# carlobaldassi/RRRMC.jl

Measured on AMD Instinct MI355X. Metric: spin-flip attempts/sec (whole node), GraphRRG N=4096 K=3 +-J standardMC beta=1.0, higher is better.
Workload: dtype u32

## Files before the change

rrrmc.jl_amd/csrc/host_sweep.hpp:

```cpp
int32_t prepare_chunk_list(rrrmc_ctx* ctx, int64_t iters, int64_t step, int C, bool* reuse_out)
{
    const bool reuse = ctx->chunks_iters == iters && ctx->chunks_step == step && ctx->chunks_C == C;
    if (!reuse) {
        std::vector<ChunkDesc> chunks;
        plan_chunk_list(iters, step, C, kWave, ctx->batch_slots_max, ctx->batch_chunks_max, ctx->batch_first_chunks, chunks, ctx->chunk_batches);
        const size_t nch_all = chunks.size();
        ctx->chunks_iters = -1;
        if (ctx->upload_pending) { HIP_TRY(ctx, hipEventSynchronize(ctx->ev_upload)); ctx->upload_pending = false; }
        if (nch_all > ctx->chunks_cap) {
            HIP_TRY(ctx, hipStreamSynchronize(ctx->stream));
            HIP_TRY(ctx, hipStreamSynchronize(ctx->plan_stream));
            free_dev(ctx->d_chunks);
            free_dev(ctx->d_chunks_alt);
            ctx->chunks_cap = 0;
            HIP_TRY(ctx, hipMalloc(&ctx->d_chunks, sizeof(ChunkDesc) * nch_all));
            if (ctx->model == RRRMC_MODEL_SPARSE_PM1) HIP_TRY(ctx, hipMalloc(&ctx->d_chunks_alt, sizeof(ChunkDesc) * nch_all));
            ctx->chunks_cap = nch_all;
        }
        if (nch_all > ctx->h_chunks_cap) {
            if (ctx->h_chunks) { (void)hipHostFree(ctx->h_chunks); ctx->h_chunks = nullptr; }
            ctx->h_chunks_cap = 0;
            HIP_TRY(ctx, hipHostMalloc(&ctx->h_chunks, sizeof(ChunkDesc) * nch_all));
            ctx->h_chunks_cap = nch_all;
        }
// ... 86 lines not shown
        if (nchunks) HIP_TRY(ctx, hipMemcpyAsync(ctx->d_chunks, ctx->h_chunks, sizeof(ChunkDesc) * nchunks, hipMemcpyHostToDevice, st));
        if (nchunks) HIP_TRY(ctx, hipMemcpyAsync(ctx->d_chunks_alt, ctx->h_chunks, sizeof(ChunkDesc) * nchunks, hipMemcpyHostToDevice, st));
        ctx->chunks_iters = iters; ctx->chunks_step = step; ctx->chunks_C = C;
        ctx->upload_pending = true;
    }
    HIP_TRY(ctx, hipEventRecord(ctx->ev_upload, st));
    if (!reuse) HIP_TRY(ctx, hipStreamWaitEvent(ctx->plan_stream, ctx->ev_upload, 0));
    for (int i = 0; i < 2; ++i)
        if (!ctx->ev_set_free[i]) HIP_TRY(ctx, hipEventCreateWithFlags(&ctx->ev_set_free[i], hipEventDisableTiming));
    const int par = ctx->plan_parity;
    auto set_of = [par](int b) -> int { return (b + par) & 1; };
    ChunkDesc* const d_chunks = (ctx->call_parity ^= 1) ? ctx->d_chunks_alt : ctx->d_chunks;

    P.spins = ctx->d_spins;
    P.table = ctx->d_table;
    P.Es = ctx->d_Es;
    P.E_cur = ctx->d_E;
    P.acc_cur = ctx->d_acc;
    P.k0 = (uint32_t)ctx->seed;
    P.k1 = (uint32_t)(ctx->seed >> 32);
    P.group0 = ctx->replica0 / 32;
    P.gbase = ctx->it_done;
    P.N = (int)N; P.C = C; P.TS = ctx->TS; P.Rpad = (int)ctx->Rpad;
    sweep_fn fn = ctx->lds_mode ? sweep_for_K((int)K, ctx->sweep_mode) : nullptr;
    BigSweepParams PB{};
    BigMaskParams PM{};
    if (ctx->big_masks) {
        std::memcpy(PM.taum, P.taum, sizeof(PM.taum));
        PM.always_mask = P.always_mask; PM.k0 = P.k0; PM.k1 = P.k1; PM.group0 = P.group0; PM.gbase = P.gbase;
        PM.cap = (uint32_t)ctx->batch_slots_max;
        PM.lgr = ctx->big_cm ? ctx->big_lgr : -1;
    }
    if (ctx->big_mode) {
        PB.spins = ctx->d_spins; PB.Es = ctx->d_Es; PB.E_cur = ctx->d_E; PB.acc_cur = ctx->d_acc;
        std::memcpy(PB.taum, P.taum, sizeof(PB.taum));
        PB.always_mask = P.always_mask; PB.k0 = P.k0; PB.k1 = P.k1; PB.group0 = P.group0; PB.gbase = P.gbase;
        PB.N = (int)N; PB.Rpad = (int)ctx->Rpad;
    }
#ifdef RRRMC_STAMPS
    if (!g_stamps) HIP_TRY(ctx, hipMalloc(&g_stamps, sizeof(unsigned long long) * 16 * (65536 + 4096)));
    P.stamps = g_stamps;
#endif
    const int nb = (int)batches.size();
    auto launch_plan = [&](int b) -> int32_t {
        const rrrmc_ctx::BatchDesc& bt = batches[b];
        const int set = set_of(b);
        if (ctx->set_used[set]) HIP_TRY(ctx, hipStreamWaitEvent(ctx->plan_stream, ctx->ev_set_free[set], 0));
        if (ctx->big_mode) {
            hipLaunchKernelGGL(plan_big_for_K((int)K), dim3((unsigned)bt.n), dim3(kPlanThreads), ctx->plan_lds_bytes, ctx->plan_stream,
                               d_chunks + bt.first, ctx->d_slots[set], ctx->d_nbrs[set], ctx->d_vecs[set], ctx->d_A, ctx->d_J, (int)N, P.k0, P.k1, P.gbase,
                               ctx->big_masks ? ctx->big_lgr : -1);
            if (ctx->big_masks) {
                PM.chunks = d_chunks + bt.first; PM.slots = ctx->d_slots[set]; PM.masks = ctx->d_masks[set];
                hipLaunchKernelGGL(big_mask_for_K((int)K), dim3((unsigned)(bt.n * (kBigChunk / kBigMaskThreads)), (unsigned)ctx->G), dim3(kBigMaskThreads), 0,
                                   ctx->plan_stream, PM);
            }
        }
        else
            hipLaunchKernelGGL(plan_for_K((int)K), dim3((unsigned)bt.n), dim3(kPlanThreads), ctx->plan_lds_bytes, ctx->plan_stream,
                               d_chunks + bt.first, ctx->d_slots[set], ctx->d_vecs[set], ctx->d_A, (int)N, C, P.k0, P.k1, P.gbase,
                               sweep_rows_for_K((int)K) * kWave);
        HIP_TRY(ctx, hipGetLastError());
        HIP_TRY(ctx, hipEventRecord(ctx->ev_plan[b], ctx->plan_stream));
// ... 48 lines not shown
```

rrrmc.jl_amd/csrc/rrrmc_hip.hip:

```cpp
#include "../../include/rrrmc_hip.h"

#include <hip/hip_runtime.h>

#include <algorithm>
#include <cmath>
#include <cstdarg>
#include <cstdio>
#include <cstdlib>
#include <cstring>
#include <string>
#include <thread>
#include <map>
#include <mutex>
#include <utility>
#include <vector>

#include "sk_kernels.hpp"
#include "sk_block_kernel.hpp"
#include "sk_hblock_kernel.hpp"
#include "rrr_kernels.hpp"
#include "quant_wave_kernel.hpp"
#include "sparse_wave_kernel.hpp"
#include "sparse_kernels.hpp"
#include "bign_kernels.hpp"
// ... 157 lines not shown
    uint32_t* rp_spins = nullptr;
    uint8_t* rp_cls = nullptr;
    uint16_t* rp_sv = nullptr;
    uint16_t* rp_spos = nullptr;
    double* wt_t = nullptr;
    uint16_t* wt_id = nullptr;
    uint16_t* wt_pos = nullptr;
    double* wt_time = nullptr;
    uint32_t wtm_calls = 0;
    bool last_call_wtm = false;
    uint32_t* eo_cmin = nullptr;
    double* eo_ftau = nullptr;
    bool last_call_eo = false;
    double* rs_buf = nullptr;
    uint32_t* rs_spins = nullptr;
    int32_t* rs_status = nullptr;

    double* pf_J = nullptr;
    unsigned long long* pf_spins = nullptr;
    double* pf_undo = nullptr;
    int32_t* pf_sites = nullptr;
    uint32_t* pf_plan = nullptr;
    int32_t* pf_status = nullptr;
    int64_t pfW = 0;
    bool pf_multi_edge = false;
    bool pf_lf_live = false;
    int8_t* db_dJ = nullptr;
    double* db_rJ = nullptr;
    uint8_t* db_cls = nullptr;
    uint16_t* db_sv = nullptr;
    uint16_t* db_spos = nullptr;
    double* db_lf = nullptr;
    double* db_undo = nullptr;
    int db_L = 0, db_ea_form = 0;
    long long db_lev_mul = 1;
    double db_lev_div = 1.0;
    bool db_cache_valid = false;
    bool q_lds_attr = false;
    bool q_cache_valid = false;
    LevTable lv{};
    long long lv_mul = 1;
    double lv_div = 1.0;
    int64_t eo_W = 0;
    int db_dElist[kDLmax] = {0};
    uint32_t* cs_spins = nullptr;
    double* cs_buf = nullptr;
// ... 344 lines not shown
    } while (0)

namespace {
int32_t post_sync_checks(rrrmc_ctx* ctx)
{
    if (ctx->debug_checks && ctx->dbg_flag) {
        int32_t fl[2] = {0, 0};
        HIP_TRY(ctx, hipMemcpy(fl, ctx->dbg_flag, sizeof fl, hipMemcpyDeviceToHost));
        HIP_TRY(ctx, hipMemset(ctx->dbg_flag, 0, sizeof fl));
        if (fl[0])
            return fail(ctx, RRRMC_ERR_STATE, "debug check failed for %d value(s), e.g. replica %d: the tracked energy / cached fields differ from "
                                              "energy(X, C) recomputed from the configuration (src/graphs/RRG.jl:229-231, SK.jl:268-273)", fl[0], fl[1]);
    }
    if (ctx->model == RRRMC_MODEL_SPARSE_F64 && ctx->pf_status && !ctx->last_call_rrr) {
        int32_t st = 0;
        HIP_TRY(ctx, hipMemcpy(&st, ctx->pf_status, sizeof st, hipMemcpyDeviceToHost));
        if (st) {
            HIP_TRY(ctx, hipMemset(ctx->pf_status, 0, sizeof st));
            ctx->results_valid = false; ctx->std_cache_live = false; ctx->pf_lf_live = false;
            return fail(ctx, RRRMC_ERR_STATE, "spf_team_kernel: a wait on the retired prefix ran into its limit (protocol failure); the call's results are void. "
                                              "RRRMC_SPF_TEAM=0 selects the single-wavefront kernel");
        }
    }
    if (ctx->last_call_rrr && (ctx->model == RRRMC_MODEL_SK_NORMAL || ctx->model == RRRMC_MODEL_SPARSE_F64) && ctx->rs_status) {
        std::vector<int32_t> stt((size_t)ctx->R);
        HIP_TRY(ctx, hipMemcpy(stt.data(), ctx->rs_status, sizeof(int32_t) * stt.size(), hipMemcpyDeviceToHost));
        for (int64_t r = 0; r < ctx->R; ++r)
            if (stt[r]) return fail(ctx, RRRMC_ERR_STATE, "replica %lld: Unrecoverable loss of precision detected in the dynamic sampler", (long long)r);
    }
    return RRRMC_OK;
}
}

extern "C" {





int32_t rrrmc_version(void) { return 100; }

const char* rrrmc_last_error(const rrrmc_ctx* ctx) { return ctx ? ctx->err.c_str() : g_create_error.c_str(); }

int32_t rrrmc_device_count(void)
{
    int n = 0;
// ... 167 lines not shown
}

void rrrmc_ctx_destroy(rrrmc_ctx* ctx)
{
    if (!ctx) return;
    if (is_multi(ctx)) {
        for (rrrmc_ctx* c : ctx->kids) rrrmc_ctx_destroy(c);
        delete ctx;
        return;
    }
    (void)hipSetDevice(ctx->device);
    if (ctx->stream) (void)hipStreamSynchronize(ctx->stream);
    free_dev(ctx->d_A); free_dev(ctx->d_J); free_dev(ctx->d_table); free_dev(ctx->d_spins);
    free_dev(ctx->d_E); free_dev(ctx->d_acc); free_dev(ctx->d_chunks); free_dev(ctx->d_chunks_alt); free_dev(ctx->d_Es);
    free_dev(ctx->d_U); free_dev(ctx->d_io);
    for (uint32_t*& l : ctx->d_color_list) free_dev(l);
    free_dev(ctx->sk_J4); free_dev(ctx->sk_blkJw); free_dev(ctx->sk_blkSites); free_dev(ctx->sk_hl);
    free_dev(ctx->sk_J); free_dev(ctx->sk_lf); free_dev(ctx->sk_lfl); free_dev(ctx->sk_move_last); free_dev(ctx->sk_spins);
    free_dev(ctx->sk_E); free_dev(ctx->sk_Es); free_dev(ctx->skb_J); free_dev(ctx->skb_lf); free_dev(ctx->skb_lfl);
    free_dev(ctx->q_spins); free_dev(ctx->q_cls); free_dev(ctx->q_sv); free_dev(ctx->q_spos); free_dev(ctx->q_st);
    free_dev(ctx->q_T); free_dev(ctx->q_z); free_dev(ctx->q_accrate); free_dev(ctx->q_stats);
    free_dev(ctx->rs_buf); free_dev(ctx->rs_spins); free_dev(ctx->rs_status);
    free_dev(ctx->rp_spins); free_dev(ctx->rp_cls); free_dev(ctx->rp_sv); free_dev(ctx->rp_spos);
    free_dev(ctx->pf_J); free_dev(ctx->pf_spins); free_dev(ctx->pf_undo); free_dev(ctx->pf_sites); free_dev(ctx->pf_plan); free_dev(ctx->pf_status);
    free_dev(ctx->db_dJ); free_dev(ctx->db_rJ); free_dev(ctx->db_cls); free_dev(ctx->db_sv); free_dev(ctx->db_spos); free_dev(ctx->db_lf); free_dev(ctx->db_undo); free_dev(ctx->db_mlast);
    free_dev(ctx->pff_table); free_dev(ctx->pff_absJ); free_dev(ctx->pff_bond_off); free_dev(ctx->pff_thr_hi); free_dev(ctx->pff_thr_lo); free_dev(ctx->pff_flags);
    free_dev(ctx->wt_t); free_dev(ctx->wt_id); free_dev(ctx->wt_pos); free_dev(ctx->wt_time);
    free_dev(ctx->smp_f); free_dev(ctx->smp_i); free_dev(ctx->cs_top);
    free_dev(ctx->q_Jf); free_dev(ctx->q_flf); free_dev(ctx->q_fundo); free_dev(ctx->q_fml);
    free_dev(ctx->eo_cmin); free_dev(ctx->eo_ftau);
    free_dev(ctx->q_Jb); free_dev(ctx->q_slf); free_dev(ctx->q_smv); free_dev(ctx->q_scur);
    free_dev(ctx->cs_spins); free_dev(ctx->cs_buf); free_dev(ctx->cs_u16);
    free_dev(ctx->snap); free_dev(ctx->d_pairs); free_dev(ctx->d_ovl); free_dev(ctx->d_qobs);
    free_dev(ctx->re_sp); free_dev(ctx->re_mu); free_dev(ctx->re_tab); free_dev(ctx->re_Eslice); free_dev(ctx->le_dist);
    free_dev(ctx->sat_off); free_dev(ctx->sat_ent); free_dev(ctx->sat_spT);
    free_dev(ctx->pc_col); free_dev(ctx->pc_row); free_dev(ctx->pc_ds); free_dev(ctx->pc_pm); free_dev(ctx->pc_mm);
    free_dev(ctx->cm_col); free_dev(ctx->cm_row); free_dev(ctx->cm_lab); free_dev(ctx->cm_ds); free_dev(ctx->cm_mk);
    for (int i = 0; i < 2; ++i) { free_dev(ctx->d_slots[i]); free_dev(ctx->d_vecs[i]); free_dev(ctx->d_nbrs[i]); free_dev(ctx->d_masks[i]); }
    free_dev(ctx->d_bigimg);
    free_dev(ctx->dbg_flag); free_dev(ctx->dbg_Ei); free_dev(ctx->dbg_lf); free_dev(ctx->dbg_lfl); free_dev(ctx->dbg_E); free_dev(ctx->dbg_ml);
    if (ctx->plan_stream) { (void)hipStreamSynchronize(ctx->plan_stream); (void)hipStreamDestroy(ctx->plan_stream); }
    if (ctx->ev_upload) (void)hipEventDestroy(ctx->ev_upload);
    for (hipEvent_t e : ctx->ev_plan) (void)hipEventDestroy(e);
    for (int i = 0; i < 2; ++i) if (ctx->ev_set_free[i]) (void)hipEventDestroy(ctx->ev_set_free[i]);
    if (ctx->h_chunks) (void)hipHostFree(ctx->h_chunks);
    for (hipEvent_t e : ctx->ev_pool) (void)hipEventDestroy(e);
    for (hipEvent_t e : ctx->ev_sweep) (void)hipEventDestroy(e);
// ... 478 lines not shown
            const int32_t rc = rrrmc_timing_total(c, &w, &l);
            if (rc) { ctx->err = c->err; return rc; }
            if (w > sw) { sw = w; nl = l; }
        }
        if (sweep_ms) *sweep_ms = sw;
        if (sweep_launches) *sweep_launches = nl;
        return RRRMC_OK;
    }
    if (!ctx) return RRRMC_ERR_INVALID_ARG;
    if (!ctx->acc_mode) return fail(ctx, RRRMC_ERR_STATE, "rrrmc_timing_accumulate(ctx, 1) has not been called");
    HIP_TRY(ctx, hipSetDevice(ctx->device));
    HIP_TRY(ctx, hipStreamSynchronize(ctx->stream));
    double sw = 0.0;
    for (size_t i = 0; i + 1 < ctx->ev_pool_used; i += 2) {
        float ms = 0.f;
        HIP_TRY(ctx, hipEventElapsedTime(&ms, ctx->ev_pool[i], ctx->ev_pool[i + 1]));
        sw += ms;
    }
    if (sweep_ms) *sweep_ms = sw;
    if (sweep_launches) *sweep_launches = (int64_t)(ctx->ev_pool_used / 2);
    return RRRMC_OK;
}

#ifdef RRRMC_STAMPS
RRRMC_API int32_t rrrmc_debug_stamps(rrrmc_ctx* ctx, int32_t group, unsigned long long* out16)
{
    HIP_TRY(ctx, hipStreamSynchronize(ctx->stream));
    HIP_TRY(ctx, hipMemcpy(out16, g_stamps + (size_t)group * 16, sizeof(unsigned long long) * 16, hipMemcpyDeviceToHost));
    return RRRMC_OK;
}
RRRMC_API int32_t rrrmc_debug_step_trace(rrrmc_ctx* ctx, unsigned long long* out)
{
    HIP_TRY(ctx, hipStreamSynchronize(ctx->stream));
    HIP_TRY(ctx, hipMemcpy(out, g_stamps + (size_t)16 * 65536, sizeof(unsigned long long) * 16 * 4096, hipMemcpyDeviceToHost));
    return RRRMC_OK;
}
#endif


int32_t rrrmc_set_coloring(rrrmc_ctx* ctx, const int32_t* color, int32_t ncolors)
{
    RRRMC_MULTI(ctx, false, rrrmc_set_coloring(c, color, ncolors));
    if (!ctx) return RRRMC_ERR_INVALID_ARG;
    if (ctx->model != RRRMC_MODEL_SPARSE_PM1) return fail(ctx, RRRMC_ERR_STATE, "colourings are for sparse +-J models");
    if (!ctx->graph_set) return fail(ctx, RRRMC_ERR_STATE, "rrrmc_set_graph has not been called");
    if (!color || ncolors < 1 || ncolors > 64) return fail(ctx, RRRMC_ERR_INVALID_ARG, "color is NULL or ncolors out of range 1..64");
    const int64_t N = ctx->N, K = ctx->K;
// ... 586 lines not shown
            }
        } else {
            hipLaunchKernelGGL(quant_standard_kernel<>, dim3(rrr_blocks(ctx->R)), dim3(rrr_tpb(ctx->R)), 0, st, P, QuantSlices::Params{});
        }
    } else {
        QwLayout ql = qw_layout(ctx->N, ctx->qW, ctx->qNk, ctx->K, (size_t)kLdsLimit, ctx->q_sk);
        if (const char* e = std::getenv("RRRMC_QUANT_WAVE_SLACK")) {
            const int64_t want = ctx->N + std::atoll(e);
            if (want >= ctx->N + 4 * kQwMinGap && want < ql.cap) ql.cap = (int)(want & ~(int64_t)3);
        }
        const char* no_wave = std::getenv("RRRMC_QUANT_NO_WAVE");
        int64_t wave_max_R = 2048;
        if (const char* e = std::getenv("RRRMC_QUANT_WAVE_MAX_R")) wave_max_R = std::atoll(e);
        const bool wave_ok = !ctx->q_skn && !ctx->q_spf && ctx->N <= 65535 && (ctx->q_sk ? ctx->qNk <= 2048 : ctx->K <= 7) && ql.cap >= ctx->N + 4 * kQwMinGap &&
                             ctx->R <= wave_max_R && !(no_wave && no_wave[0] == '1');
        const size_t lds = rrr_quant_lds_bytes(ctx->N, ctx->qW, ctx->qNk, ctx->K);
        const char* no_lds = std::getenv("RRRMC_QUANT_NO_LDS");
        if (wave_ok) {
            HIP_TRY(ctx, raise_lds_attr(ctx->q_sk ? reinterpret_cast<const void*>(rrr_quant_wave_kernel<true>) : reinterpret_cast<const void*>(rrr_quant_wave_kernel<false>), ql.bytes));
            QwExtra X{};
            X.cap = ql.cap; X.off_spos = (uint32_t)ql.off_spos; X.off_sv = (uint32_t)ql.off_sv; X.off_A = (uint32_t)ql.off_A;
            X.off_J = (uint32_t)ql.off_J; X.off_rng = (uint32_t)ql.off_rng; X.off_tab = (uint32_t)ql.off_tab;
#ifdef RRRMC_STAMPS
            if (!g_stamps) HIP_TRY(ctx, hipMalloc(&g_stamps, sizeof(unsigned long long) * 16 * (65536 + 4096)));
            X.stamps = g_stamps;
#endif
            if (ctx->q_sk) hipLaunchKernelGGL(rrr_quant_wave_kernel<true>, dim3((unsigned)ctx->R), dim3(kRrrThreads), ql.bytes, st, P, X);
            else hipLaunchKernelGGL(rrr_quant_wave_kernel<false>, dim3((unsigned)ctx->R), dim3(kRrrThreads), ql.bytes, st, P, X);
        } else if (!ctx->q_skn && !ctx->q_spf && ctx->N <= 65535 && rrr_tpb(ctx->R) == 1 && lds <= (size_t)kLdsLimit && !(no_lds && no_lds[0] == '1')) {
            if (!ctx->q_lds_attr) {
                HIP_TRY(ctx, raise_lds_attr(reinterpret_cast<const void*>(rrr_quant_kernel<true>), lds));
                ctx->q_lds_attr = true;
            }
            hipLaunchKernelGGL(rrr_quant_kernel<true>, dim3((unsigned)ctx->R), dim3(kRrrThreads), lds, st, P, QuantSlices::Params{});
        } else {
            hipLaunchKernelGGL(rrr_quant_kernel<false>, dim3(rrr_blocks(ctx->R)), dim3(rrr_tpb(ctx->R)), 0, st, P, QuantSlices::Params{});
        }
    }
    HIP_TRY(ctx, hipGetLastError());
    HIP_TRY(ctx, hipEventRecord(ctx->ev_sweep[1], st));
    if (ctx->q_pat && ctx->debug_checks) { rc = quant_pat_check(ctx, P); if (rc) return rc; }
    HIP_TRY(ctx, hipEventRecord(ctx->ev_end, st));
    ctx->sweep_launches = 1;
    ctx->nsamp = nsamp;
    ctx->it_done += (uint64_t)iters;
    if (!standard) smp_commit(ctx, 1, iters);
    ctx->results_valid = true;
// ... 1008 lines not shown
```

rrrmc.jl_amd/csrc/sparse_kernels.hpp:

```cpp
#pragma once
#include <hip/hip_runtime.h>
#include <stdint.h>

#include "philox.hpp"
#include "host_plan.hpp"

namespace rrrmc {

constexpr int kWave = 64;
#ifndef RRRMC_SWEEP_THREADS
#define RRRMC_SWEEP_THREADS 1024
#endif
constexpr int kSweepThreads = RRRMC_SWEEP_THREADS;
#ifndef RRRMC_FIXER_WAVE
#define RRRMC_FIXER_WAVE 14
#endif
#ifndef RRRMC_TALLY_WAVE
#define RRRMC_TALLY_WAVE 1
#endif
constexpr int kConsumerWave = 0, kTallyWave = 1, kFixerWave = RRRMC_FIXER_WAVE;
constexpr int kSwTallyWave = RRRMC_TALLY_WAVE;
__host__ __device__ constexpr int sw_producer_index(int wave)
{
    int pw = 0;
    for (int w = 0; w < wave; ++w) pw += (w != kConsumerWave && w != kSwTallyWave && w != kFixerWave) ? 1 : 0;
    return pw;
}
constexpr int kProducerWaves = kSweepThreads / kWave - 3;
constexpr int kMaxChunkSlots = 2048;
constexpr int kProducerTasksMax = (kMaxChunkSlots / kWave + kProducerWaves - 1) / kProducerWaves;
constexpr int kProducerBlocks = 3;
constexpr int kLeftMax = 128;
constexpr int kSwBlocks = 3;
constexpr int kSwFixBlocks = 0;
constexpr int kSwLeftMax = 128;
#ifndef RRRMC_PLAN_THREADS
#define RRRMC_PLAN_THREADS 512
#endif
constexpr int kPlanThreads = RRRMC_PLAN_THREADS;
constexpr int kMaxK = 7;
#ifndef RRRMC_ROWS
#define RRRMC_ROWS 14
#endif
template <int K> constexpr int sweep_rows() { return K <= 3 ? RRRMC_ROWS : (K == 4 ? (RRRMC_ROWS < 8 ? RRRMC_ROWS : 8) : (RRRMC_ROWS < 4 ? RRRMC_ROWS : 4)); }

__device__ __forceinline__ uint32_t wave_count_by_key(uint32_t* counter, uint32_t key, bool active)
{
    uint32_t slot = 0u;
    unsigned long long todo = __ballot(active);
    while (todo) {
        const int leader = __builtin_ctzll(todo);
        const uint32_t k0 = (uint32_t)__builtin_amdgcn_readlane((int)key, leader);
        const unsigned long long same = __ballot(active && key == k0);
// ... 130 lines not shown
        const uint32_t l = act ? (uint32_t)s_lvl[t] : 0u;
        const uint32_t pos = wave_count_by_key(s_cur, l, act);
        if (act) slots[cd.slot_base + s_start[l] + pos] = (uint32_t)s_site[t] | ((uint32_t)t << 16);
    }
}

struct SweepParams {
    uint32_t* spins;
    const uint16_t* table;
    const ChunkDesc* chunks;
    const uint32_t* slots;
    const uint32_t* vecs;
    int32_t* Es;
    int32_t* E_cur;
    int64_t* acc_cur;
    uint32_t taum[64 * 4];
    uint32_t always_mask;
    uint32_t k0, k1;
    uint32_t group0;
    int64_t sample0;
    uint64_t gbase;
    int N, C, TS, Rpad, nchunks;
    unsigned long long* stamps;
};

template <int K> struct SweepCfg {
    static constexpr int NT = (K + 1) / 2;
    static constexpr int NW = NT + (K + 2) / 2;
    static constexpr int NQ = (NW + 3) / 4;
    static constexpr int NS = K <= 1 ? 2 : (K <= 3 ? 3 : 4);
};

struct LeftList {
    uint32_t* count;
    uint32_t* slot;
    uint32_t* lt;
    uint32_t* eq;
};

template <int NT> __device__ __forceinline__ bool any_set(const uint32_t (&eq)[NT])
{
    uint32_t u = 0u;
#pragma unroll
    for (int n = 0; n < NT; ++n) u |= eq[n];
    return u != 0u;
}

template <int NT>
__device__ __forceinline__ void refine_block(uint32_t (&lt)[NT], uint32_t (&eq)[NT], const Philox4& o, uint32_t pb, const uint32_t* __restrict__ taum)
{
#pragma unroll
    for (int n = 0; n < NT; ++n) {
        uint32_t x[4];
#pragma unroll
        for (int j = 0; j < 4; ++j) {
            const uint32_t tm = taum[(pb * 4 + j) * 4 + n];
            x[j] = bitop3<0x20>(eq[n], o.w[j], tm);
            eq[n] = bitop3<0x90>(eq[n], o.w[j], tm);
        }
        lt[n] = (lt[n] | x[0] | x[1]) | (x[2] | x[3]);
    }
}

template <int K, int MODE>
__device__ __forceinline__ void produce_chunk(const SweepParams& P, const ChunkDesc& cd, uint4* __restrict__ desc,
                                              const uint16_t* __restrict__ tbl, const LeftList& left, int pw, int lane, uint32_t group,
                                              const uint32_t (&slots)[kProducerTasksMax])
{
    constexpr int NT = SweepCfg<K>::NT, NQ = SweepCfg<K>::NQ;
    const int C = P.C;
    const int ntask = ((int)cd.count + kWave - 1) / kWave;
#pragma unroll
    for (int j = 0; j < kProducerTasksMax; ++j) {
        const int task = pw + j * kProducerWaves;
        if (task >= ntask) break;
        const int p = task * kWave + lane;
        const bool live = p < (int)cd.count;
        const uint32_t slot = slots[j];
        const uint32_t site = slot & 0xffffu;
        const uint64_t g = P.gbase + cd.g0 + (uint64_t)(slot >> 16);

        uint32_t f[NQ * 4];
#pragma unroll
        for (int q = 0; q < NQ * 4; ++q) f[q] = 0u;
        {
            uint32_t off[K + 2];
            off[0] = MODE == 3 ? site : MODE == 2 ? 2u * site : site * 8u;
            off[K + 1] = 0u;
            const uint16_t* row = tbl + (size_t)site * P.TS;
            if constexpr (K <= 4) {
                const uint2 r = *reinterpret_cast<const uint2*>(row);
                const uint32_t e[4] = {r.x & 0xffffu, r.x >> 16, r.y & 0xffffu, r.y >> 16};
#pragma unroll
                for (int k = 0; k < K; ++k) off[1 + k] = e[k];
            } else {
                const uint4 r = *reinterpret_cast<const uint4*>(row);
                const uint32_t e[8] = {r.x & 0xffffu, r.x >> 16, r.y & 0xffffu, r.y >> 16, r.z & 0xffffu, r.z >> 16, r.w & 0xffffu, r.w >> 16};
#pragma unroll
// ... 470 lines not shown
    uint4* desc = reinterpret_cast<uint4*>(sp + (((MODE == 3 ? 1 : 2) * N + 128 + 3) & ~3));
    uint4* tal = desc + 3 * NQ * C;
    uint32_t* leftmem = reinterpret_cast<uint32_t*>(tal + 2 * (C + kWave));
    constexpr int kLeftBuf = kSwLeftMax * (1 + 2 * SweepCfg<K>::NT);
    constexpr int kLeftAll = 4 + 2 * kLeftBuf;
    const uint16_t* tbl = MODE >= 1 ? P.table : reinterpret_cast<const uint16_t*>(leftmem + kLeftAll);

    const int tid = threadIdx.x, lane = tid & 63;
    const int wave = __builtin_amdgcn_readfirstlane(tid >> 6);
    const uint32_t group = P.group0 + blockIdx.x;
    uint32_t* gsp = P.spins + (size_t)blockIdx.x * N;

    for (int x = tid; x < N; x += kSweepThreads) {
        const uint32_t w = gsp[x];
        if constexpr (MODE == 3) sp[x] = w;
        else *reinterpret_cast<uint2*>(sp + 2 * x) = make_uint2(w, ~w);
    }
    if constexpr (MODE == 0) {
        uint16_t* tbl_w = reinterpret_cast<uint16_t*>(leftmem + kLeftAll);
        for (int q = tid; q < N * P.TS; q += kSweepThreads) tbl_w[q] = P.table[q];
    }
    if (tid < 4) leftmem[tid] = 0u;
    __syncthreads();
    auto left_list = [&](int c) {
        uint32_t* m = leftmem + 4 + (c & 1) * kLeftBuf;
        LeftList l;
        l.count = leftmem + (c % 3); l.slot = m; l.lt = m + kSwLeftMax; l.eq = m + kSwLeftMax * (1 + SweepCfg<K>::NT);
        return l;
    };

    const int nsteps = P.nchunks + 3;
    const int tal_stride = C + kWave;
#ifdef RRRMC_STAMPS
    unsigned long long busy = 0;
#define RRRMC_T0 const unsigned long long t_in = __builtin_amdgcn_s_memtime();
#define RRRMC_T1 { const unsigned long long dt_ = __builtin_amdgcn_s_memtime() - t_in; busy += dt_; \
        if (blockIdx.x == 0 && lane == 0 && P.stamps && c < 4096) P.stamps[16 * 65536 + c * 16 + wave] = dt_; }
#else
#define RRRMC_T0
#define RRRMC_T1
#endif
    if (wave == kConsumerWave) {
        __builtin_amdgcn_s_setprio(3);
        ChunkDesc ca{}, cb{}, cc{};
        uint32_t va = 0u, vb = 0u;
        for (int c = 0; c < nsteps; ++c) {
            RRRMC_T0
            ca = cb; va = vb;
            cb = cc;
            vb = (c >= 1 && c - 1 < P.nchunks && (uint32_t)lane < cb.nvec) ? P.vecs[cb.slot_base + lane] : 0u;
            if (c < P.nchunks) cc = P.chunks[c];
#ifndef RRRMC_ABLATE_CONSUME
            if (c >= 2 && c - 2 < P.nchunks)
                consume_chunk<K, MODE>(P, ca, desc + ((c - 2) % 3) * NQ * C, sp, tal + ((c - 2) & 1) * tal_stride, lane, va);
#endif
            RRRMC_T1
            __syncthreads();
        }
    } else if (wave == kSwTallyWave) {
        __builtin_amdgcn_s_setprio(2);
        TransposeConsts tc;
        tc.init(lane);
        TallyState<NS> ts;
        tally_reset<NS>(ts);
        TallyDrain<NS, K> dr;
        tally_reset<NS>(dr.set);
        dr.tot[0] = 0u; dr.tot[1] = 0u; dr.phase = NS; dr.emit = false; dr.sample = 0;
        int32_t E_run = 0;
        int64_t A_run = 0;
        if (lane < 32) { E_run = P.E_cur[blockIdx.x * 32 + lane]; A_run = P.acc_cur[blockIdx.x * 32 + lane]; }
        int64_t ns = P.sample0;
        const uint32_t grp_per_chunk = (uint32_t)((C + 8 * kWave - 1) / (8 * kWave));
        ChunkDesc ta{}, tb{};
        for (int c = 0; c < nsteps; ++c) {
            RRRMC_T0
            ta = tb;
            if (c >= 2 && c - 2 < P.nchunks) tb = P.chunks[c - 2];
#ifndef RRRMC_ABLATE_TALLY
            if (c >= 3) {
                const ChunkDesc cd = ta;
                const bool sample = (cd.flags & kChunkSampleBefore) != 0;
                if (sample || ts.ngrp + grp_per_chunk > (1u << kTallyHi) - 1u) {
                    dr.run_to_end(P, tc, lane, E_run, A_run);
                    dr.set = ts;
                    tally_reset<NS>(ts);
                    dr.tot[0] = 0u; dr.tot[1] = 0u; dr.phase = 0;
                    dr.emit = sample; dr.sample = ns;
                    if (sample) ns += 1;
                }
                if (dr.phase < NS) {
                    dr.step(tc);
                    if (dr.phase == NS) dr.finish(P, lane, E_run, A_run);
                }
                tally_chunk<NS, K>(ts, cd, tal + ((c - 3) & 1) * tal_stride, lane);
            }
#endif
            RRRMC_T1
            __syncthreads();
        }
        dr.run_to_end(P, tc, lane, E_run, A_run);
        dr.set = ts;
        dr.tot[0] = 0u; dr.tot[1] = 0u; dr.phase = 0; dr.emit = false;
        dr.run_to_end(P, tc, lane, E_run, A_run);
        if (lane < 32) { P.E_cur[blockIdx.x * 32 + lane] = E_run; P.acc_cur[blockIdx.x * 32 + lane] = A_run; }
    } else if (wave == kFixerWave) {
        ChunkDesc fa{}, fb{};
        for (int c = 0; c < nsteps; ++c) {
            RRRMC_T0
            fa = fb;
            if (c < P.nchunks) fb = P.chunks[c];
            if (lane == 0) leftmem[(c + 1) % 3] = 0u;
            if (c >= 1 && c - 1 < P.nchunks) fix_tasks<K>(P, fa, desc + ((c - 1) % 3) * NQ * C, left_list(c - 1), lane, group, 0);
            RRRMC_T1
            __syncthreads();
        }
    } else {
        const int pw = sw_producer_index(wave);
        ChunkDesc cdp{}, cd0{}, cd1{}, cd2{};
        uint32_t sl0[kProducerTasksMax], sl1[kProducerTasksMax];
#pragma unroll
        for (int j = 0; j < kProducerTasksMax; ++j) { sl0[j] = 0u; sl1[j] = 0u; }
        auto fetch_slots = [&](const ChunkDesc& cd, uint32_t (&sl)[kProducerTasksMax]) {
#pragma unroll
            for (int j = 0; j < kProducerTasksMax; ++j) {
                const int p = (pw + j * kProducerWaves) * kWave + lane;
                sl[j] = p < (int)cd.count ? P.slots[cd.slot_base + p] : 0u;
            }
        };
        if (P.nchunks > 0) { cd1 = P.chunks[0]; fetch_slots(cd1, sl1); }
        if (P.nchunks > 1) cd2 = P.chunks[1];
        for (int c = 0; c < nsteps; ++c) {
            RRRMC_T0
            cdp = cd0;
            cd0 = cd1;
#pragma unroll
            for (int j = 0; j < kProducerTasksMax; ++j) sl0[j] = sl1[j];
            cd1 = cd2;
            if (c + 1 < P.nchunks) fetch_slots(cd1, sl1);
            if (c + 2 < P.nchunks) cd2 = P.chunks[c + 2];
#ifndef RRRMC_ABLATE_PRODUCE
            if constexpr (kSwLeftMax > 2 * kWave)
                if (c >= 1 && c - 1 < P.nchunks) fix_tasks<K>(P, cdp, desc + ((c - 1) % 3) * NQ * C, left_list(c - 1), lane, group, 1 + pw);
            if (c < P.nchunks) produce_chunk<K, MODE>(P, cd0, desc + (c % 3) * NQ * C, tbl, left_list(c), pw, lane, group, sl0);
#endif
            RRRMC_T1
            __syncthreads();
        }
    }
#ifdef RRRMC_STAMPS
    if (lane == 0 && P.stamps) P.stamps[blockIdx.x * 16 + wave] = busy;
#endif
#undef RRRMC_T0
#undef RRRMC_T1
    __syncthreads();
    int tid_wb = tid;
    asm volatile("" : "+v"(tid_wb));
    for (int x = tid_wb; x < N; x += kSweepThreads) gsp[x] = sp[MODE == 3 ? x : 2 * x];
}

__global__ __launch_bounds__(256) void energy_kernel(const uint32_t* __restrict__ spins, const int32_t* __restrict__ A,
                                                     const int8_t* __restrict__ J, int N, int K, int32_t* __restrict__ E_out,
                                                     uint8_t* __restrict__ nun)
{
    __shared__ uint32_t sU[32];
    const int tid = threadIdx.x, r = tid & 31, part = tid >> 5;
    const uint32_t* sp = spins + (size_t)blockIdx.x * N;
    if (tid < 32) sU[tid] = 0;
    __syncthreads();
    uint32_t U = 0;
    for (int x = part; x < N; x += 8) {
        const uint32_t s = (sp[x] >> r) & 1u;
        uint32_t n = 0;
        for (int k = 0; k < K; ++k) {
            const uint32_t sy = (sp[A[(size_t)x * K + k]] >> r) & 1u;
            n += s ^ sy ^ (J[(size_t)x * K + k] < 0 ? 1u : 0u);
        }
        U += n;
// ... 164 lines not shown
```

Baseline: 4171 billion.

## Replace per-chunk block barriers with LDS progress flags between wave roles

The sweep kernel's consumer, tally, fixer and producer wavefronts no longer meet at a __syncthreads every chunk. Each wave now publishes its progress counter in LDS and polls only the counters of the roles it depends on, with fixed lags. Producer tasks are also dealt round-robin across chunks through a rotating offset, so the leftover tasks of a partly filled chunk land on different waves. Chunk descriptors are read through the constant address space, and the wave priority is raised only around the consume and tally work. The change adds a poll limit with an abort flag that is reported to the host as a protocol failure, and it risks races or spin overhead if the lags are wrong.

```diff
diff --git a/rrrmc.jl_amd/csrc/host_sweep.hpp b/rrrmc.jl_amd/csrc/host_sweep.hpp
--- a/rrrmc.jl_amd/csrc/host_sweep.hpp
+++ b/rrrmc.jl_amd/csrc/host_sweep.hpp
@@ -132,6 +132,11 @@
     P.group0 = ctx->replica0 / 32;
     P.gbase = ctx->it_done;
     P.N = (int)N; P.C = C; P.TS = ctx->TS; P.Rpad = (int)ctx->Rpad;
+    if (ctx->lds_mode && !ctx->sw_status) {
+        HIP_TRY(ctx, hipMalloc(&ctx->sw_status, sizeof(int32_t)));
+        HIP_TRY(ctx, hipMemsetAsync(ctx->sw_status, 0, sizeof(int32_t), st));
+    }
+    P.status = ctx->sw_status;
     sweep_fn fn = ctx->lds_mode ? sweep_for_K((int)K, ctx->sweep_mode) : nullptr;
     BigSweepParams PB{};
     BigMaskParams PM{};
@@ -148,7 +153,7 @@
         PB.N = (int)N; PB.Rpad = (int)ctx->Rpad;
     }
 #ifdef RRRMC_STAMPS
-    if (!g_stamps) HIP_TRY(ctx, hipMalloc(&g_stamps, sizeof(unsigned long long) * 16 * (65536 + 4096)));
+    if (!g_stamps) HIP_TRY(ctx, hipMalloc(&g_stamps, sizeof(unsigned long long) * 16 * (2 * 65536 + 4096)));
     P.stamps = g_stamps;
 #endif
     const int nb = (int)batches.size();
diff --git a/rrrmc.jl_amd/csrc/rrrmc_hip.hip b/rrrmc.jl_amd/csrc/rrrmc_hip.hip
--- a/rrrmc.jl_amd/csrc/rrrmc_hip.hip
+++ b/rrrmc.jl_amd/csrc/rrrmc_hip.hip
@@ -203,6 +203,7 @@
     int32_t* pf_sites = nullptr;
     uint32_t* pf_plan = nullptr;
     int32_t* pf_status = nullptr;
+    int32_t* sw_status = nullptr;
     int64_t pfW = 0;
     bool pf_multi_edge = false;
     bool pf_lf_live = false;
@@ -593,6 +594,15 @@
                                               "RRRMC_SPF_TEAM=0 selects the single-wavefront kernel");
         }
     }
+    if (ctx->model == RRRMC_MODEL_SPARSE_PM1 && ctx->sw_status) {
+        int32_t st = 0;
+        HIP_TRY(ctx, hipMemcpy(&st, ctx->sw_status, sizeof st, hipMemcpyDeviceToHost));
+        if (st) {
+            HIP_TRY(ctx, hipMemset(ctx->sw_status, 0, sizeof st));
+            ctx->results_valid = false;
+            return fail(ctx, RRRMC_ERR_STATE, "sweep_kernel: a wait on another wavefront's progress ran into its limit (protocol failure); the call's results are void");
+        }
+    }
     if (ctx->last_call_rrr && (ctx->model == RRRMC_MODEL_SK_NORMAL || ctx->model == RRRMC_MODEL_SPARSE_F64) && ctx->rs_status) {
         std::vector<int32_t> stt((size_t)ctx->R);
         HIP_TRY(ctx, hipMemcpy(stt.data(), ctx->rs_status, sizeof(int32_t) * stt.size(), hipMemcpyDeviceToHost));
@@ -806,7 +816,7 @@
     free_dev(ctx->q_T); free_dev(ctx->q_z); free_dev(ctx->q_accrate); free_dev(ctx->q_stats);
     free_dev(ctx->rs_buf); free_dev(ctx->rs_spins); free_dev(ctx->rs_status);
     free_dev(ctx->rp_spins); free_dev(ctx->rp_cls); free_dev(ctx->rp_sv); free_dev(ctx->rp_spos);
-    free_dev(ctx->pf_J); free_dev(ctx->pf_spins); free_dev(ctx->pf_undo); free_dev(ctx->pf_sites); free_dev(ctx->pf_plan); free_dev(ctx->pf_status);
+    free_dev(ctx->pf_J); free_dev(ctx->pf_spins); free_dev(ctx->pf_undo); free_dev(ctx->pf_sites); free_dev(ctx->pf_plan); free_dev(ctx->pf_status); free_dev(ctx->sw_status);
     free_dev(ctx->db_dJ); free_dev(ctx->db_rJ); free_dev(ctx->db_cls); free_dev(ctx->db_sv); free_dev(ctx->db_spos); free_dev(ctx->db_lf); free_dev(ctx->db_undo); free_dev(ctx->db_mlast);
     free_dev(ctx->pff_table); free_dev(ctx->pff_absJ); free_dev(ctx->pff_bond_off); free_dev(ctx->pff_thr_hi); free_dev(ctx->pff_thr_lo); free_dev(ctx->pff_flags);
     free_dev(ctx->wt_t); free_dev(ctx->wt_id); free_dev(ctx->wt_pos); free_dev(ctx->wt_time);
@@ -1331,7 +1341,25 @@
     return RRRMC_OK;
 }
 
+RRRMC_API int32_t rrrmc_debug_chunk_list(rrrmc_ctx* ctx, int64_t iters, int64_t step, int32_t* C_out, uint32_t* counts, int64_t cap, int64_t* n_out)
+{
+    if (!ctx || is_multi(ctx) || ctx->model != RRRMC_MODEL_SPARSE_PM1 || iters < 0 || step < 1 || !n_out) return RRRMC_ERR_INVALID_ARG;
+    std::vector<ChunkDesc> chunks;
+    std::vector<rrrmc_ctx::BatchDesc> batches;
+    plan_chunk_list(iters, step, ctx->C, kWave, ctx->batch_slots_max, ctx->batch_chunks_max, ctx->batch_first_chunks, chunks, batches);
+    if (C_out) *C_out = ctx->C;
+    *n_out = (int64_t)chunks.size();
+    for (size_t i = 0; i < chunks.size() && (int64_t)i < cap; ++i) counts[i] = chunks[i].count;
+    return RRRMC_OK;
+}
+
 #ifdef RRRMC_STAMPS
+RRRMC_API int32_t rrrmc_debug_stamps_wait(rrrmc_ctx* ctx, int32_t group, unsigned long long* out16)
+{
+    HIP_TRY(ctx, hipStreamSynchronize(ctx->stream));
+    HIP_TRY(ctx, hipMemcpy(out16, g_stamps + (size_t)16 * (65536 + 4096) + (size_t)group * 16, sizeof(unsigned long long) * 16, hipMemcpyDeviceToHost));
+    return RRRMC_OK;
+}
 RRRMC_API int32_t rrrmc_debug_stamps(rrrmc_ctx* ctx, int32_t group, unsigned long long* out16)
 {
     HIP_TRY(ctx, hipStreamSynchronize(ctx->stream));
@@ -1964,7 +1992,7 @@
             X.cap = ql.cap; X.off_spos = (uint32_t)ql.off_spos; X.off_sv = (uint32_t)ql.off_sv; X.off_A = (uint32_t)ql.off_A;
             X.off_J = (uint32_t)ql.off_J; X.off_rng = (uint32_t)ql.off_rng; X.off_tab = (uint32_t)ql.off_tab;
 #ifdef RRRMC_STAMPS
-            if (!g_stamps) HIP_TRY(ctx, hipMalloc(&g_stamps, sizeof(unsigned long long) * 16 * (65536 + 4096)));
+            if (!g_stamps) HIP_TRY(ctx, hipMalloc(&g_stamps, sizeof(unsigned long long) * 16 * (2 * 65536 + 4096)));
             X.stamps = g_stamps;
 #endif
             if (ctx->q_sk) hipLaunchKernelGGL(rrr_quant_wave_kernel<true>, dim3((unsigned)ctx->R), dim3(kRrrThreads), ql.bytes, st, P, X);
diff --git a/rrrmc.jl_amd/csrc/sparse_kernels.hpp b/rrrmc.jl_amd/csrc/sparse_kernels.hpp
--- a/rrrmc.jl_amd/csrc/sparse_kernels.hpp
+++ b/rrrmc.jl_amd/csrc/sparse_kernels.hpp
@@ -2,8 +2,11 @@
 #include <hip/hip_runtime.h>
 #include <stdint.h>
 
+#include <type_traits>
+
 #include "philox.hpp"
 #include "host_plan.hpp"
+#include "sweep_flow.hpp"
 
 namespace rrrmc {
 
@@ -29,6 +32,13 @@
 constexpr int kProducerWaves = kSweepThreads / kWave - 3;
 constexpr int kMaxChunkSlots = 2048;
 constexpr int kProducerTasksMax = (kMaxChunkSlots / kWave + kProducerWaves - 1) / kProducerWaves;
+#ifndef RRRMC_DEAL
+#define RRRMC_DEAL 0
+#endif
+constexpr DealTable kDeal = (RRRMC_DEAL == 1 && kProducerWaves == 13) ? deal_weighted13() : deal_plain(kProducerWaves);
+static_assert(deal_valid(kDeal, kProducerWaves), "every task of the deal has a producer wave");
+static_assert(kMaxChunkSlots / kWave <= 32 && deal_most_per_chunk(kDeal, kProducerWaves, kMaxChunkSlots / kWave) <= kProducerTasksMax,
+              "the deal gives a producer wave more tasks of one chunk than its slot registers hold");
 constexpr int kProducerBlocks = 3;
 constexpr int kLeftMax = 128;
 constexpr int kSwBlocks = 3;
@@ -205,7 +215,29 @@
     uint64_t gbase;
     int N, C, TS, Rpad, nchunks;
     unsigned long long* stamps;
+    int32_t* status;
 };
+
+constexpr int kFlowAbortWord = 16;
+constexpr int kFlowPollLimit = 1 << 22;
+#ifndef RRRMC_FLOW_NAP
+#define RRRMC_FLOW_NAP 1
+#endif
+template <int Q> __device__ __forceinline__ uint64_t deal_mask_of(int pw)
+{
+    constexpr uint64_t m = deal_mask(kDeal, Q);
+    if constexpr (Q == 0) return m;
+    else return pw == Q ? m : deal_mask_of<Q - 1>(pw);
+}
+
+__device__ __forceinline__ ChunkDesc chunk_desc(const ChunkDesc* p)
+{
+    typedef const ChunkDesc __attribute__((address_space(4))) * cptr;
+    const cptr q = (cptr)(uintptr_t)p;
+    ChunkDesc d;
+    d.g0 = q->g0; d.count = q->count; d.slot_base = q->slot_base; d.nvec = q->nvec; d.flags = q->flags;
+    return d;
+}
 
 template <int K> struct SweepCfg {
     static constexpr int NT = (K + 1) / 2;
@@ -247,16 +279,15 @@
 
 template <int K, int MODE>
 __device__ __forceinline__ void produce_chunk(const SweepParams& P, const ChunkDesc& cd, uint4* __restrict__ desc,
-                                              const uint16_t* __restrict__ tbl, const LeftList& left, int pw, int lane, uint32_t group,
-                                              const uint32_t (&slots)[kProducerTasksMax])
+                                              const uint16_t* __restrict__ tbl, const LeftList& left, const int (&tasks)[kProducerTasksMax], int lane,
+                                              uint32_t group, const uint32_t (&slots)[kProducerTasksMax])
 {
     constexpr int NT = SweepCfg<K>::NT, NQ = SweepCfg<K>::NQ;
     const int C = P.C;
-    const int ntask = ((int)cd.count + kWave - 1) / kWave;
 #pragma unroll
     for (int j = 0; j < kProducerTasksMax; ++j) {
-        const int task = pw + j * kProducerWaves;
-        if (task >= ntask) break;
+        const int task = tasks[j];
+        if (task < 0) break;
         const int p = task * kWave + lane;
         const bool live = p < (int)cd.count;
         const uint32_t slot = slots[j];
@@ -773,43 +804,78 @@
     }
     if (tid < 4) leftmem[tid] = 0u;
     __syncthreads();
+    int32_t* flow = reinterpret_cast<int32_t*>(sp + (((MODE == 3 ? 1 : 2) * N + 3) & ~3));
+    if (tid < 32) flow[tid] = 0;
+    __syncthreads();
     auto left_list = [&](int c) {
-        uint32_t* m = leftmem + 4 + (c & 1) * kLeftBuf;
+        uint32_t* m = leftmem + 4 + flow_left_ring(c) * kLeftBuf;
         LeftList l;
-        l.count = leftmem + (c % 3); l.slot = m; l.lt = m + kSwLeftMax; l.eq = m + kSwLeftMax * (1 + SweepCfg<K>::NT);
+        l.count = leftmem + flow_count_ring(c); l.slot = m; l.lt = m + kSwLeftMax; l.eq = m + kSwLeftMax * (1 + SweepCfg<K>::NT);
         return l;
     };
-
-    const int nsteps = P.nchunks + 3;
+    static_assert(kSwLeftMax <= 2 * kWave, "the hand-over below lets only the fixer wave read a chunk's leftover list");
+
+    const int nch = P.nchunks;
     const int tal_stride = C + kWave;
+    constexpr int kWaves = kSweepThreads / kWave;
+    auto role_of = [](int w) { return w == kConsumerWave ? kFlowConsumer : w == kSwTallyWave ? kFlowTally : w == kFixerWave ? kFlowFixer : kFlowProducer; };
+    auto flow_wait = [&](auto role, int c) -> bool {
+        int l = lane;
+        asm volatile("" : "+v"(l));
+        const int fl = l & 31;
+        const int lag = fl < kWaves ? flow_lag(decltype(role)::value, role_of(fl)) : kFlowNone;
+        const int need = c + lag;
+        for (int polls = 0;;) {
+            const int32_t v = __hip_atomic_load(flow + fl, __ATOMIC_RELAXED, __HIP_MEMORY_SCOPE_WORKGROUP);
+            if (__all(v >= need)) break;
+            if (__any(fl == kFlowAbortWord && v != 0)) return false;
+            if (++polls > kFlowPollLimit) {
+                if (lane == 0) __hip_atomic_store(flow + kFlowAbortWord, 1, __ATOMIC_RELAXED, __HIP_MEMORY_SCOPE_WORKGROUP);
+                return false;
+            }
+            __builtin_amdgcn_s_sleep(RRRMC_FLOW_NAP);
+        }
+        __builtin_amdgcn_fence(__ATOMIC_ACQUIRE, "workgroup");
+        return true;
+    };
+    auto flow_publish = [&](int done) {
+        __builtin_amdgcn_fence(__ATOMIC_RELEASE, "workgroup");
+        if (lane == 0) __hip_atomic_store(flow + wave, done, __ATOMIC_RELAXED, __HIP_MEMORY_SCOPE_WORKGROUP);
+    };
 #ifdef RRRMC_STAMPS
-    unsigned long long busy = 0;
-#define RRRMC_T0 const unsigned long long t_in = __builtin_amdgcn_s_memtime();
-#define RRRMC_T1 { const unsigned long long dt_ = __builtin_amdgcn_s_memtime() - t_in; busy += dt_; \
+    unsigned long long busy = 0, waited = 0, t_mark = __builtin_amdgcn_s_memtime();
+    auto lap = [&](unsigned long long& acc) { const unsigned long long now = __builtin_amdgcn_s_memtime(), dt = now - t_mark; acc += dt; t_mark = now; return dt; };
+#define RRRMC_LAP_BUSY lap(busy);
+#define RRRMC_LAP_WAIT lap(waited);
+#define RRRMC_LAP_WORK { const unsigned long long dt_ = lap(busy); \
         if (blockIdx.x == 0 && lane == 0 && P.stamps && c < 4096) P.stamps[16 * 65536 + c * 16 + wave] = dt_; }
 #else
-#define RRRMC_T0
-#define RRRMC_T1
+#define RRRMC_LAP_BUSY
+#define RRRMC_LAP_WAIT
+#define RRRMC_LAP_WORK
 #endif
     if (wave == kConsumerWave) {
-        __builtin_amdgcn_s_setprio(3);
         ChunkDesc ca{}, cb{}, cc{};
         uint32_t va = 0u, vb = 0u;
-        for (int c = 0; c < nsteps; ++c) {
-            RRRMC_T0
+        if (nch > 0) { cb = chunk_desc(P.chunks + (0)); vb = (uint32_t)lane < cb.nvec ? P.vecs[cb.slot_base + lane] : 0u; }
+        if (nch > 1) cc = chunk_desc(P.chunks + (1));
+        for (int c = 0; c < nch; ++c) {
+            RRRMC_LAP_BUSY
+            if (!flow_wait(std::integral_constant<int, kFlowConsumer>{}, c)) break;
+            RRRMC_LAP_WAIT
             ca = cb; va = vb;
             cb = cc;
-            vb = (c >= 1 && c - 1 < P.nchunks && (uint32_t)lane < cb.nvec) ? P.vecs[cb.slot_base + lane] : 0u;
-            if (c < P.nchunks) cc = P.chunks[c];
+            vb = (c + 1 < nch && (uint32_t)lane < cb.nvec) ? P.vecs[cb.slot_base + lane] : 0u;
+            if (c + 2 < nch) cc = chunk_desc(P.chunks + (c + 2));
 #ifndef RRRMC_ABLATE_CONSUME
-            if (c >= 2 && c - 2 < P.nchunks)
-                consume_chunk<K, MODE>(P, ca, desc + ((c - 2) % 3) * NQ * C, sp, tal + ((c - 2) & 1) * tal_stride, lane, va);
+            __builtin_amdgcn_s_setprio(3);
+            consume_chunk<K, MODE>(P, ca, desc + flow_desc_ring(c) * NQ * C, sp, tal + flow_tal_ring(c) * tal_stride, lane, va);
+            __builtin_amdgcn_s_setprio(0);
 #endif
-            RRRMC_T1
-            __syncthreads();
+            flow_publish(c + 1);
+            RRRMC_LAP_WORK
         }
     } else if (wave == kSwTallyWave) {
-        __builtin_amdgcn_s_setprio(2);
         TransposeConsts tc;
         tc.init(lane);
         TallyState<NS> ts;
@@ -823,12 +889,17 @@
         int64_t ns = P.sample0;
         const uint32_t grp_per_chunk = (uint32_t)((C + 8 * kWave - 1) / (8 * kWave));
         ChunkDesc ta{}, tb{};
-        for (int c = 0; c < nsteps; ++c) {
-            RRRMC_T0
+        bool alive = true;
+        if (nch > 0) tb = chunk_desc(P.chunks + (0));
+        for (int c = 0; c < nch; ++c) {
+            RRRMC_LAP_BUSY
+            alive = alive && flow_wait(std::integral_constant<int, kFlowTally>{}, c);
+            RRRMC_LAP_WAIT
             ta = tb;
-            if (c >= 2 && c - 2 < P.nchunks) tb = P.chunks[c - 2];
+            if (c + 1 < nch) tb = chunk_desc(P.chunks + (c + 1));
 #ifndef RRRMC_ABLATE_TALLY
-            if (c >= 3) {
+            if (alive) {
+                __builtin_amdgcn_s_setprio(2);
                 const ChunkDesc cd = ta;
                 const bool sample = (cd.flags & kChunkSampleBefore) != 0;
                 if (sample || ts.ngrp + grp_per_chunk > (1u << kTallyHi) - 1u) {
@@ -843,11 +914,12 @@
                     dr.step(tc);
                     if (dr.phase == NS) dr.finish(P, lane, E_run, A_run);
                 }
-                tally_chunk<NS, K>(ts, cd, tal + ((c - 3) & 1) * tal_stride, lane);
+                tally_chunk<NS, K>(ts, cd, tal + flow_tal_ring(c) * tal_stride, lane);
+                __builtin_amdgcn_s_setprio(0);
             }
 #endif
-            RRRMC_T1
-            __syncthreads();
+            flow_publish(c + 1);
+            RRRMC_LAP_WORK
         }
         dr.run_to_end(P, tc, lane, E_run, A_run);
         dr.set = ts;
@@ -856,54 +928,67 @@
         if (lane < 32) { P.E_cur[blockIdx.x * 32 + lane] = E_run; P.acc_cur[blockIdx.x * 32 + lane] = A_run; }
     } else if (wave == kFixerWave) {
         ChunkDesc fa{}, fb{};
-        for (int c = 0; c < nsteps; ++c) {
-            RRRMC_T0
+        if (nch > 0) fb = chunk_desc(P.chunks + (0));
+        for (int c = 0; c < nch; ++c) {
+            RRRMC_LAP_BUSY
+            if (!flow_wait(std::integral_constant<int, kFlowFixer>{}, c)) break;
+            RRRMC_LAP_WAIT
             fa = fb;
-            if (c < P.nchunks) fb = P.chunks[c];
-            if (lane == 0) leftmem[(c + 1) % 3] = 0u;
-            if (c >= 1 && c - 1 < P.nchunks) fix_tasks<K>(P, fa, desc + ((c - 1) % 3) * NQ * C, left_list(c - 1), lane, group, 0);
-            RRRMC_T1
-            __syncthreads();
+            if (c + 1 < nch) fb = chunk_desc(P.chunks + (c + 1));
+            fix_tasks<K>(P, fa, desc + flow_desc_ring(c) * NQ * C, left_list(c), lane, group, 0);
+            if (lane == 0) leftmem[flow_count_ring(c)] = 0u;
+            flow_publish(c + 1);
+            RRRMC_LAP_WORK
         }
     } else {
         const int pw = sw_producer_index(wave);
-        ChunkDesc cdp{}, cd0{}, cd1{}, cd2{};
+        const uint64_t mine = deal_mask_of<kProducerWaves - 1>(pw);
+        ChunkDesc cd0{}, cd1{}, cd2{};
         uint32_t sl0[kProducerTasksMax], sl1[kProducerTasksMax];
-#pragma unroll
-        for (int j = 0; j < kProducerTasksMax; ++j) { sl0[j] = 0u; sl1[j] = 0u; }
-        auto fetch_slots = [&](const ChunkDesc& cd, uint32_t (&sl)[kProducerTasksMax]) {
+        int tk0[kProducerTasksMax], tk1[kProducerTasksMax];
+#pragma unroll
+        for (int j = 0; j < kProducerTasksMax; ++j) { sl0[j] = 0u; sl1[j] = 0u; tk0[j] = -1; tk1[j] = -1; }
+        int t0 = 0;
+        auto fetch_slots = [&](const ChunkDesc& cd, uint32_t (&sl)[kProducerTasksMax], int (&tk)[kProducerTasksMax]) {
+            const int ntask = ((int)cd.count + kWave - 1) / kWave;
+            uint32_t bits = deal_tasks(mine, t0, ntask);
+            t0 = deal_advance(kDeal, t0, ntask);
 #pragma unroll
             for (int j = 0; j < kProducerTasksMax; ++j) {
-                const int p = (pw + j * kProducerWaves) * kWave + lane;
-                sl[j] = p < (int)cd.count ? P.slots[cd.slot_base + p] : 0u;
+                const int task = bits ? (int)__builtin_ctz(bits) : -1;
+                bits &= bits - 1u;
+                tk[j] = task;
+                const int p = task * kWave + lane;
+                sl[j] = (task >= 0 && p < (int)cd.count) ? P.slots[cd.slot_base + p] : 0u;
             }
         };
-        if (P.nchunks > 0) { cd1 = P.chunks[0]; fetch_slots(cd1, sl1); }
-        if (P.nchunks > 1) cd2 = P.chunks[1];
-        for (int c = 0; c < nsteps; ++c) {
-            RRRMC_T0
-            cdp = cd0;
+        if (nch > 0) { cd1 = chunk_desc(P.chunks + (0)); fetch_slots(cd1, sl1, tk1); }
+        if (nch > 1) cd2 = chunk_desc(P.chunks + (1));
+        for (int c = 0; c < nch; ++c) {
+            RRRMC_LAP_BUSY
+            if (!flow_wait(std::integral_constant<int, kFlowProducer>{}, c)) break;
+            RRRMC_LAP_WAIT
             cd0 = cd1;
 #pragma unroll
-            for (int j = 0; j < kProducerTasksMax; ++j) sl0[j] = sl1[j];
+            for (int j = 0; j < kProducerTasksMax; ++j) { sl0[j] = sl1[j]; tk0[j] = tk1[j]; }
             cd1 = cd2;
-            if (c + 1 < P.nchunks) fetch_slots(cd1, sl1);
-            if (c + 2 < P.nchunks) cd2 = P.chunks[c + 2];
+            if (c + 1 < nch) fetch_slots(cd1, sl1, tk1);
+            if (c + 2 < nch) cd2 = chunk_desc(P.chunks + (c + 2));
 #ifndef RRRMC_ABLATE_PRODUCE
-            if constexpr (kSwLeftMax > 2 * kWave)
-                if (c >= 1 && c - 1 < P.nchunks) fix_tasks<K>(P, cdp, desc + ((c - 1) % 3) * NQ * C, left_list(c - 1), lane, group, 1 + pw);
-            if (c < P.nchunks) produce_chunk<K, MODE>(P, cd0, desc + (c % 3) * NQ * C, tbl, left_list(c), pw, lane, group, sl0);
+            produce_chunk<K, MODE>(P, cd0, desc + flow_desc_ring(c) * NQ * C, tbl, left_list(c), tk0, lane, group, sl0);
 #endif
-            RRRMC_T1
-            __syncthreads();
+            flow_publish(c + 1);
+            RRRMC_LAP_WORK
         }
     }
 #ifdef RRRMC_STAMPS
-    if (lane == 0 && P.stamps) P.stamps[blockIdx.x * 16 + wave] = busy;
+    if (lane == 0 && P.stamps) { P.stamps[blockIdx.x * 16 + wave] = busy; P.stamps[16 * (65536 + 4096) + blockIdx.x * 16 + wave] = waited; }
 #endif
-#undef RRRMC_T0
-#undef RRRMC_T1
-    __syncthreads();
+#undef RRRMC_LAP_BUSY
+#undef RRRMC_LAP_WAIT
+#undef RRRMC_LAP_WORK
+    __syncthreads();
+    if (tid == 0 && flow[kFlowAbortWord] != 0 && P.status) *P.status = 1;
     int tid_wb = tid;
     asm volatile("" : "+v"(tid_wb));
     for (int x = tid_wb; x < N; x += kSweepThreads) gsp[x] = sp[MODE == 3 ? x : 2 * x];
diff --git a/rrrmc.jl_amd/csrc/sweep_flow.hpp b/rrrmc.jl_amd/csrc/sweep_flow.hpp
--- /dev/null
+++ b/rrrmc.jl_amd/csrc/sweep_flow.hpp
@@ -0,0 +1,83 @@
+#pragma once
+#include <stdint.h>
+
+namespace rrrmc {
+
+enum : int { kFlowProducer = 0, kFlowFixer = 1, kFlowConsumer = 2, kFlowTally = 3 };
+constexpr int kFlowNone = -(1 << 30);
+
+constexpr int flow_desc_ring(int c) { return c % 3; }
+constexpr int flow_left_ring(int c) { return c & 1; }
+constexpr int flow_count_ring(int c) { return c % 3; }
+constexpr int flow_tal_ring(int c) { return c & 1; }
+
+#ifndef RRRMC_FLOW_WEAKEN
+#define RRRMC_FLOW_WEAKEN 0
+#endif
+
+constexpr int flow_lag(int by, int of)
+{
+    constexpr int W = RRRMC_FLOW_WEAKEN;
+    if (by == kFlowProducer && of == kFlowConsumer) return (W == 1 || W == 5) ? kFlowNone : -2;
+    if (by == kFlowProducer && of == kFlowFixer) return (W == 1 || W == 6) ? kFlowNone : -1;
+    if (by == kFlowFixer && of == kFlowProducer) return W == 2 ? kFlowNone : 1;
+    if (by == kFlowConsumer && of == kFlowFixer) return (W == 3 || W == 7) ? kFlowNone : 1;
+    if (by == kFlowConsumer && of == kFlowTally) return (W == 3 || W == 8) ? kFlowNone : -1;
+    if (by == kFlowTally && of == kFlowConsumer) return W == 4 ? kFlowNone : 1;
+    return kFlowNone;
+}
+constexpr bool flow_ready(int by, int of, int c, int32_t progress_of) { return progress_of >= c + flow_lag(by, of); }
+
+constexpr int kDealPeriodMax = 32;
+struct DealTable { int period; int8_t owner[kDealPeriodMax]; };
+
+constexpr DealTable deal_plain(int P)
+{
+    DealTable t{};
+    t.period = P;
+    for (int i = 0; i < kDealPeriodMax; ++i) t.owner[i] = (int8_t)(i < P ? i : 0);
+    return t;
+}
+constexpr DealTable deal_weighted13()
+{
+    DealTable t{};
+    t.period = 32;
+    for (int i = 0; i < 26; ++i) t.owner[i] = (int8_t)(i % 13);
+    const int8_t extra[6] = {0, 1, 3, 4, 5, 8};
+    for (int i = 0; i < 6; ++i) t.owner[26 + i] = extra[i];
+    return t;
+}
+
+constexpr uint64_t deal_mask(const DealTable& t, int pw)
+{
+    uint64_t m = 0;
+    for (int b = 0; b < 64; ++b)
+        if (t.owner[b % t.period] == pw) m |= 1ull << b;
+    return m;
+}
+constexpr uint32_t deal_tasks(uint64_t mask, int t0, int ntask)
+{
+    return (uint32_t)(mask >> t0) & (ntask >= 32 ? 0xffffffffu : ((1u << ntask) - 1u));
+}
+constexpr int deal_advance(const DealTable& t, int t0, int ntask) { return (t0 + ntask) % t.period; }
+constexpr int deal_most_per_chunk(const DealTable& t, int P, int max_tasks)
+{
+    int most = 0;
+    for (int pw = 0; pw < P; ++pw)
+        for (int t0 = 0; t0 < t.period; ++t0) {
+            const uint32_t bits = deal_tasks(deal_mask(t, pw), t0, max_tasks);
+            int n = 0;
+            for (int b = 0; b < 32; ++b) n += (int)((bits >> b) & 1u);
+            most = n > most ? n : most;
+        }
+    return most;
+}
+constexpr bool deal_valid(const DealTable& t, int P)
+{
+    if (t.period < 1 || t.period > kDealPeriodMax) return false;
+    for (int i = 0; i < t.period; ++i)
+        if (t.owner[i] < 0 || t.owner[i] >= P) return false;
+    return true;
+}
+
+}
```

Result: slower. 3408 billion (-18.3%).
